# ut-amrl/nautilus

Measured on AMD Instinct MI355X. Metric: loop-closure candidate pairs/sec (1081-beam), higher is better.
Workload: dtype u16

## Files before the change

nautilus_amd/csrc/nhip_bnb.hip:

```cpp
#include <atomic>
#include <mutex>
#include <type_traits>
#include <vector>

#ifndef NHIP_BNB_INSTR
#define NHIP_BNB_INSTR 0
#endif
#if NHIP_BNB_INSTR
#define csm_bnb_kernel csm_bnb_kernel_instr
#define csm_bnb_rot_kernel csm_bnb_rot_kernel_instr
#define launchers_product launchers_instr
#define BNB_STATS(P) ((P).stats)
#define BNB_TIMELINE(P) ((P).timeline)
#else
#define BNB_STATS(P) (static_cast<unsigned long long *>(nullptr))
#define BNB_TIMELINE(P) (static_cast<unsigned long long *>(nullptr))
#endif

#include "nhip_bnb_params.h"
#include "nhip_bnb_wave.h"
#include "nhip_bnb_origin.h"
#include "nhip_bnb_bounds.h"
#include "nhip_bnb_exact.h"

// ... 239 lines not shown
      for (int q = 0; q < 12; q++) sb[q] = 0xffffffffu;
    }
    uint32_t mk0 = 0u, mk1 = 0u;
#pragma unroll 1
    for (int t = 0; t < len; t++) {
      const int b = b0 + t;
      if (b < 64) m0 &= ~(1ull << b);
      else m1 &= ~(1ull << (b - 64));
      const uint32_t ub = (uint32_t)__builtin_amdgcn_readlane((int)(b < 64 ? u0 : u1), b & 63);
      if (ub < best_sum_cached<GLOBAL>(best, bcopy)) continue;
      const uint32_t s0 = t == 0 ? sb[0] : (t == 1 ? sb[4] : sb[8]), s1 = t == 0 ? sb[1] : (t == 1 ? sb[5] : sb[9]);
      const uint32_t s2 = t == 0 ? sb[2] : (t == 1 ? sb[6] : sb[10]), s3 = t == 0 ? sb[3] : (t == 1 ? sb[7] : sb[11]);
      if (BNB_STATS(P)) t_mark = clock64();
      process_candidate_c<CB, GLOBAL, PAIR>(P, rsrc, pitch8, rsrc16, org, nch, C.n_pts, k, Y, X0 + t, s0, s1, s2, s3, lane, best,
                                      bcopy, n_work, t, mk0, mk1);
      if (BNB_STATS(P)) clk.eval += clock64() - t_mark;
      if (done && wave_leader(lane)) done[b] = 0u;
    }
    if (PAIR && (mk0 | mk1) != 0u) {
      if (BNB_STATS(P)) t_mark = clock64();
      strip_sub_blocks<CB, GLOBAL>(P, rsrc, pitch8, rsrc16, org, nch, C.n_pts, k, Y, X0, sb, mk0, mk1, lane, best, bcopy, n_work);
      if (BNB_STATS(P)) clk.eval += clock64() - t_mark;
    }
  }
}

__device__ __forceinline__ void read_entry(const RotEntry *ent, int32_t *pair, int32_t *k, unsigned long long *m0,
                                           unsigned long long *m1) {
  const unsigned long long w0 = ent->w[0], w1 = ent->w[1], w2 = ent->w[2], w3 = ent->w[3];
  *pair = (int32_t)(w0 >> 24);
  *k = (int32_t)(w0 & 0xffffffull);
  *m0 = w1 | (w2 << 41);
  *m1 = (w2 >> 23) | (w3 << 18);
}

__device__ __forceinline__ void pair_context(const BnbParams &P, int32_t pair, PairCtx *C) {
  const int32_t src = P.pair_src[pair], slot = P.pair_slot[pair];
  const int32_t beg = P.offsets[src];
  C->grid = P.grids + (size_t)slot * P.slot_bytes;
  C->pts = P.xy + beg;
  C->n_pts = P.offsets[src + 1] - beg;
  C->cx = P.pair_origin ? P.pair_origin[2 * pair] : 0;
  C->cy = P.pair_origin ? P.pair_origin[2 * pair + 1] : 0;
  C->pair = pair;
}

template <int CB, bool POOL_LDS, bool BY_ROT, bool SPLIT = false>
__global__ __launch_bounds__(SPLIT ? 64 * SPLIT_WAVES : BNB_THREADS, SPLIT ? SPLIT_WAVES / 2 : 4) void csm_bnb_kernel(BnbParams P) {
  constexpr int WAVES = SPLIT ? SPLIT_WAVES : BNB_WAVES, THREADS = 64 * WAVES;
  constexpr int QSPACE = lds_qspace(SPLIT);
  extern __shared__ __align__(16) uint8_t smem[];
  uint8_t *s_pool = smem;
  uint32_t *s_org = reinterpret_cast<uint32_t *>(smem);
  uint32_t *s_U = reinterpret_cast<uint32_t *>(smem + P.lds_first);
  unsigned long long *s_queue = reinterpret_cast<unsigned long long *>(s_U + (size_t)P.n_theta * 128);
  LdsTail *s_tail = reinterpret_cast<LdsTail *>(s_queue + QSPACE);
  unsigned long long *s_best = &s_tail->best, *s_slow = &s_tail->slow;
  uint32_t *s_cnt = s_tail->cnt, *s_qn = s_cnt + LDS_QN, *s_qhead = s_cnt + LDS_QHEAD, *s_top = &s_tail->top;
  uint32_t *s_list = reinterpret_cast<uint32_t *>(s_queue);
  static_assert(BNB_WAVES * LIST_ENTRIES * 4 <= QCAP * 4, "the run lists fit the first half of the queue");
  unsigned long long *s_kmax = s_queue + (SPLIT ? WAVES * LIST_ENTRIES / 2 : QCAP / 2);
  uint32_t *s_order = reinterpret_cast<uint32_t *>(s_kmax + MAX_ROT);
  static_assert(SPLIT_WAVES * LIST_ENTRIES * 4 + MAX_ROT * 12 <= QSPACE_SPLIT * 8 && MAX_ROT * 12 <= QCAP * 4, "lists, maxima and order fit");

  const uint32_t bid = blockIdx.x;
  const int32_t pair = (int32_t)((bid & 7u) * (uint32_t)P.pairs_per_xcd + (bid >> 3));
  if ((int32_t)(bid >> 3) >= P.pairs_per_xcd || pair >= P.n_pairs) return;
  const int lane = threadIdx.x & 63, wave = threadIdx.x >> 6;

  int32_t src = P.pair_src[pair], slot = P.pair_slot[pair];
  const bool ids_ok = pair_ids_ok(P.ids, src, slot, pair + P.pair_base, threadIdx.x == 0);
  if (!ids_ok) src = slot = 0;
  const int32_t beg = ids_ok ? P.offsets[src] : 0, n_pts = ids_ok ? P.offsets[src + 1] - beg : 0;
  const float2 *pts = P.xy + beg;
  const uint8_t *grid = P.grids + (size_t)slot * P.slot_bytes;
  const int32_t cx = P.pair_origin ? P.pair_origin[2 * pair] : 0;
  const int32_t cy = P.pair_origin ? P.pair_origin[2 * pair + 1] : 0;
  const bool centre_ok = (abs(cx) + P.hx <= P.max_shift) && (abs(cy) + P.hy <= P.max_shift);
  if (BY_ROT != (n_pts <= 64 * OCL && (uint32_t)P.rows < ORG_LIMIT && !P.general_all)) return;

  const int32_t gfloor = gate_floor(P.gate, n_pts);
  const unsigned long long fkey = gate_floor_key(gfloor);
  unsigned long long *const stats_g = NHIP_BNB_INSTR ? P.stats : nullptr;
  const long long t_start = BNB_STATS(P) ? clock64() : 0;
  if (BNB_TIMELINE(P) && threadIdx.x == 0 && pair < BNB_STATS_PAIRS) BNB_TIMELINE(P)[4 * pair] = wall_clock64();
  if (threadIdx.x == 0) {
    *s_slow = 0ull;
    *s_best = fkey;
    s_cnt[0] = s_cnt[3] = s_cnt[4] = s_cnt[5] = 0u;
    s_top[0] = 0u;
    *s_qn = 0u;
    *s_qhead = 0u;
  }
  if (!centre_ok || n_pts <= 0) {
    if (threadIdx.x == 0) P.keys[pair] = fkey;
    return;
  }
  const RotationTerms terms = rotation_terms_of_wave<WAVES>(P, pair, wave, lane);
  if (POOL_LDS) {
    const uint4 *gp = reinterpret_cast<const uint4 *>(grid + P.grid_bytes + P.skip_bytes);
    uint4 *sp = reinterpret_cast<uint4 *>(s_pool);
    const int32_t n16 = (int32_t)(P.pool_bytes / 16);
    for (int32_t i = threadIdx.x; i < n16; i += 4 * THREADS) {
      uint4 v[4];
#pragma unroll
      for (int j = 0; j < 4; j++) v[j] = gp[min(i + j * THREADS, n16 - 1)];
#pragma unroll
      for (int j = 0; j < 4; j++)
        if (i + j * THREADS < n16) sp[i + j * THREADS] = v[j];
    }
  }
  const __amdgpu_buffer_rsrc_t prs = uniform_rsrc(grid + P.grid_bytes + P.skip_bytes, P.pool_bytes);
  float cfs, sfs;
  rotation_of(terms, &cfs, &sfs);
  __syncthreads();

  const uint32_t scale = CB == 1 ? 1u : 257u;
  unsigned long long wbest = 0ull;
  PointSlots slots;
  prime_slots(pts, wave < P.n_theta ? n_pts : 0, lane, slots);
  int32_t mine = 0;
  for (int32_t k = wave; k < P.n_theta; k += WAVES, mine++) {
    const float cf = __int_as_float(__builtin_amdgcn_readlane(__float_as_int(cfs), mine));
    const float sf = __int_as_float(__builtin_amdgcn_readlane(__float_as_int(sfs), mine));
    uint32_t umax = 0u;
    uint32_t tot[2];
    coarse_rotation<POOL_LDS>(P, s_pool, prs, pts, n_pts, slots, cf, sf, cx, cy, lane, s_list + wave * LIST_ENTRIES, tot);
    if (lane < 128 - NB * NB) s_U[k * 128 + NB * NB + lane] = 0u;
#pragma unroll
    for (int i = 0; i < 2; i++) {
      int Y, X;
      if (!slot_block(lane + 64 * i, &Y, &X)) continue;
      const uint32_t u = (Y < P.nby && X < P.nbx) ? tot[i] * scale : 0u;
      const int b = NB * Y + X;
      s_U[k * 128 + b] = u;
      umax = u > umax ? u : umax;
      const unsigned long long cand = ((unsigned long long)u << 32) | (uint32_t)((k << 8) | b);
      wbest = cand > wbest ? cand : wbest;
    }
    if (BY_ROT) {
      umax = wave_max(umax);
      if (wave_leader(lane)) s_kmax[k] = ((unsigned long long)umax << 32) | (uint32_t)k;
    }
  }
  wbest = wave_max_u64(wbest);
  if (gfloor > 0) {
    if (wave_leader(lane)) atomicMax(s_top, (uint32_t)(wbest >> 32));
    __syncthreads();
    if (*s_top < (uint32_t)gfloor) {
      if (threadIdx.x == 0) {
        P.keys[pair] = fkey;
        if (stats_g) {
          atomicAdd(&stats_g[1], (unsigned long long)(P.n_theta * P.nbx * P.nby));
          atomicAdd(&stats_g[15], 1ull);
        }
      }
      return;
    }
    if ((uint32_t)(wbest >> 32) < (uint32_t)gfloor) wbest = 0ull;
  }
  uint32_t n_work[N_WORK] = {};
  PairCtx C;
  C.grid = grid;
  C.pts = pts;
  C.n_pts = n_pts;
  C.cx = cx;
  C.cy = cy;
  C.pair = pair;
  if (BY_ROT) {
    __syncthreads();
    uint32_t *org = s_org + wave * ORG_WAVE + lane;
    PhaseClocks clk = {0, 0, 0, 0u, 0u, 0u};
    long long t_busy = 0, t_wall = 0;
    const long long t_phase1 = BNB_STATS(P) ? clock64() : 0;
    if (BNB_TIMELINE(P) && threadIdx.x == 0 && pair < BNB_STATS_PAIRS) BNB_TIMELINE(P)[4 * pair + 1] = wall_clock64();
    const uint32_t xcd = bid & 7u;
    bool handed_over = false;
    enum { SEED, OWN };
    int state = SEED;
    bool heavy = false;
    for (;;) {
      bool have = false;
      int32_t k = 0;
      uint32_t u0 = 0u, u1 = 0u;
      unsigned long long m0 = 0ull, m1 = 0ull;
      uint32_t *done = nullptr;
      if (state == SEED) {
        if ((uint32_t)(wbest >> 32) != 0u) {
          const int32_t v = (int32_t)(wbest & 0xffu);
          const uint32_t ub = (uint32_t)(wbest >> 32);
          k = (int32_t)((uint32_t)wbest >> 8);
          u0 = v == lane ? ub : 0u;
          u1 = v == lane + 64 ? ub : 0u;
          m0 = v < 64 ? 1ull << v : 0ull;
          m1 = v < 64 ? 0ull : 1ull << (v - 64);
          done = s_U + k * 128;
          have = true;
        }
      } else if (state == OWN) {
        const int32_t rank = (int32_t)wave_fetch_add(s_qhead, 1u, lane);
        if (rank >= P.n_theta) break;
        k = (int32_t)s_order[rank];
        u0 = s_U[k * 128 + lane];
        u1 = s_U[k * 128 + 64 + lane];
        const uint32_t bsum = best_sum<false>(s_best);
        m0 = __ballot(u0 != 0u && u0 >= bsum);
        m1 = __ballot(u1 != 0u && u1 >= bsum && lane + 64 < NB * NB);
        if ((m0 | m1) == 0ull) continue;
        if (heavy && (uint32_t)rank >= P.keep_ranks) {
          const uint32_t lx = (xcd + (uint32_t)rank) & 7u;
          const uint32_t e = wave_fetch_add(P.rot_count + 8 * lx, 1u, lane);
          if (e < P.rot_cap) {
            if (lane < 4) {
              const unsigned long long M41 = (1ull << 41) - 1ull;
              const unsigned long long word = lane == 0   ? ((unsigned long long)(uint32_t)pair << 24) | (uint32_t)k
                                              : lane == 1 ? (m0 & M41)
                                              : lane == 2 ? ((m0 >> 41) | (m1 << 23)) & M41
                                                          : (m1 >> 18);
              P.rot_list[(size_t)lx * P.rot_cap + e].w[lane] = word;
            }
            handed_over = true;
            continue;
          }
        }
        have = true;
      }
      if (have) rotation_pass<CB, false, false>(P, C, k, u0, u1, m0, m1, lane, s_best, done, org, n_work, clk);
      if (state == SEED) {
        __syncthreads();
        if (BNB_TIMELINE(P) && threadIdx.x == 0 && pair < BNB_STATS_PAIRS) BNB_TIMELINE(P)[4 * pair + 2] = wall_clock64();
        if (BNB_STATS(P)) {
          t_busy = clock64();
          t_wall = wall_clock64();
        }
        for (int32_t kk = threadIdx.x; kk < P.n_theta; kk += THREADS) {
          const unsigned long long mine = s_kmax[kk];
          int32_t rank = 0;
          for (int32_t j = 0; j < P.n_theta; j++) rank += s_kmax[j] > mine ? 1 : 0;
          s_order[rank] = (uint32_t)kk;
        }
        if (P.rot_list || SPLIT) {
          const uint32_t bsum = best_sum<false>(s_best);
          uint32_t mine = 0u;
          for (int32_t kk = wave; kk < P.n_theta; kk += WAVES) {
            const uint32_t c0 = s_U[kk * 128 + lane], c1 = s_U[kk * 128 + 64 + lane];
            mine += (uint32_t)__builtin_popcountll(__ballot(c0 != 0u && c0 >= bsum)) +
                    (uint32_t)__builtin_popcountll(__ballot(c1 != 0u && c1 >= bsum && lane + 64 < NB * NB));
          }
          if (wave_leader(lane)) atomicAdd(s_qn, mine);
        }
        __syncthreads();
        if (SPLIT) {
          const uint32_t bsum = best_sum<false>(s_best);
          uint32_t *rows = P.ps_rows + (size_t)pair * (size_t)P.n_theta * 128u;
          uint32_t live = 0u;
          for (int32_t r = wave; r < P.n_theta; r += WAVES) {
            const uint32_t kk = s_order[r];
            const uint32_t kmax = (uint32_t)(s_kmax[kk] >> 32);
            if (kmax == 0u || kmax < bsum) break;
            live = (uint32_t)r + 1u;
            const uint32_t w1 = lane == 62 ? kmax : (lane == 63 ? kk : s_U[kk * 128 + 64 + lane]);
            rows[(size_t)r * 128u + lane] = s_U[kk * 128 + lane];
            rows[(size_t)r * 128u + 64 + lane] = w1;
          }
          if (live && wave_leader(lane)) atomicMax(s_qhead, live);
          __syncthreads();
          if (threadIdx.x == 0) {
            P.ps_count[pair] = *s_qn;
            P.ps_live[pair] = *s_qhead;
            P.ps_next[pair] = 0u;
          }
          break;
        }
        heavy = P.rot_list && *s_qn >= P.heavy_min;
        state = OWN;
      }
    }
    if (BNB_STATS(P) && lane == 0) {
      const long long now = clock64();
      atomicAdd(&BNB_STATS(P)[4], (unsigned long long)(now - t_busy));
      atomicAdd(&BNB_STATS(P)[11], (unsigned long long)(wall_clock64() - t_wall));
      flush_stats(BNB_STATS(P), nullptr, pair, &clk);
      atomicMax(s_slow, (unsigned long long)(now - t_busy));
      if (wave == 0) {
        atomicAdd(&BNB_STATS(P)[9], (unsigned long long)(t_busy - t_phase1));
        atomicAdd(&BNB_STATS(P)[10], (unsigned long long)(t_phase1 - t_start));
        if (handed_over) atomicAdd(&BNB_STATS(P)[12], 1ull);
      }
    }
  } else {
  if ((uint32_t)(wbest >> 32) != 0u) {
      const int32_t k = (int32_t)((uint32_t)wbest >> 8), v = (int32_t)(wbest & 0xffu);
      const int Y = v / NB, X = v - NB * Y;
      float cf, sf;
      rotation_k(P, pair, k, &cf, &sf);
      const unsigned long long key = eval_block<CB>(P, grid, pts, n_pts, cf, sf, cx, cy, k, Y, X, lane);
      if (wave_leader(lane)) {
        atomicMax(s_best, key);
        s_U[k * 128 + v] = 0u;
      }
      n_work[0]++;
    }
    __syncthreads();
    for (int32_t k = wave; k < P.n_theta; k += BNB_WAVES) {
  #pragma unroll
      for (int i = 0; i < 2; i++) {
        const uint32_t u = s_U[k * 128 + lane + 64 * i];
        const uint32_t bsum = (uint32_t)(*(volatile unsigned long long *)s_best >> 32);
        bool cand = u != 0u && u >= bsum;
        const unsigned long long m = __ballot(cand);
        if (m == 0ull) continue;
        const uint32_t base = wave_fetch_add(s_qn, (uint32_t)__builtin_popcountll(m), lane);
        const uint32_t pos = base + (uint32_t)__builtin_popcountll(m & ((1ull << lane) - 1ull));
        const unsigned long long entry = ((unsigned long long)u << 32) | (uint32_t)((k << 8) | (lane + 64 * i));
        if (cand && pos < (uint32_t)QCAP) s_queue[pos] = entry;
        unsigned long long over = __ballot(cand && pos >= (uint32_t)QCAP);
        while (over) {
          const int j = (int)__builtin_ctzll(over);
          over &= over - 1ull;
          const uint32_t lo = (uint32_t)__builtin_amdgcn_readlane((int)(uint32_t)entry, j);
          const uint32_t hi = (uint32_t)__builtin_amdgcn_readlane((int)(uint32_t)(entry >> 32), j);
          if (hi >= best_sum<false>(s_best))
            process_candidate<CB>(P, C, (int32_t)(lo >> 8), (int32_t)(lo & 0xffu), lane, s_best, n_work);
        }
      }
    }
    __syncthreads();
    {
      const uint32_t qn = min(*s_qn, (uint32_t)QCAP);
      for (;;) {
        const uint32_t i = wave_fetch_add(s_qhead, 1u, lane);
        if (i >= qn) break;
        const unsigned long long entry = s_queue[i];
        if ((uint32_t)(entry >> 32) >= best_sum<false>(s_best))
          process_candidate<CB>(P, C, (int32_t)((uint32_t)entry >> 8), (int32_t)(entry & 0xffu), lane, s_best, n_work);
      }
    }
}
  if (stats_g && lane == 0) {
    atomicAdd(&s_cnt[0], n_work[0]);
    atomicAdd(&s_cnt[3], n_work[1]);
    atomicAdd(&s_cnt[4], n_work[2]);
    atomicAdd(&s_cnt[5], n_work[3]);
    flush_stats(stats_g, nullptr, pair, nullptr, n_work + 4);
  }
  __syncthreads();
  if (threadIdx.x == 0) {
    P.keys[pair] = *s_best;
    if (BNB_TIMELINE(P) && pair < BNB_STATS_PAIRS) {
      uint32_t hw;
      asm volatile("s_getreg_b32 %0, hwreg(HW_REG_HW_ID)" : "=s"(hw));
      uint32_t xcc;
      asm volatile("s_getreg_b32 %0, hwreg(HW_REG_XCC_ID)" : "=s"(xcc));
      BNB_TIMELINE(P)[4 * pair + 3] = (wall_clock64() & 0xfffffffffffull) | ((unsigned long long)((hw >> 8) & 0xffu) << 44) |
                                      ((unsigned long long)(xcc & 0xfu) << 52);
    }
    if (BNB_STATS(P) && BY_ROT) atomicAdd(&BNB_STATS(P)[8], *s_slow);
    if (stats_g) {
      const uint32_t n_all[4] = {s_cnt[0], s_cnt[3], s_cnt[4], s_cnt[5]};
      flush_stats(stats_g, n_all, pair, nullptr);
      atomicAdd(&stats_g[1], (unsigned long long)(P.n_theta * P.nbx * P.nby));
    }
  }
}
// ... 262 lines not shown
```

nautilus_amd/csrc/nhip_bnb_bounds.h:

```cpp
#pragma once
#include <type_traits>

#include "nhip_bnb_origin.h"

namespace nhip {
namespace {

constexpr uint32_t LANE_WEIGHT = 64u;

struct PointSlots {
  float2 q0, q1;
};
__device__ __forceinline__ void prime_slots(const float2 *pts, int32_t n_pts, int lane, PointSlots &S) {
  S.q0 = S.q1 = make_float2(0.f, 0.f);
  if (n_pts > 0) {
    const int32_t last = n_pts - 1;
    S.q0 = pts[min(lane, last)];
    __builtin_amdgcn_sched_barrier(0);
    S.q1 = pts[min(64 + lane, last)];
  }
}

template <bool POOL_LDS>
__device__ __forceinline__ void coarse_rotation(const BnbParams &P, const uint8_t *pool, __amdgpu_buffer_rsrc_t prs,
                                                const float2 *pts, int32_t n_pts, PointSlots &S, float cf, float sf,
                                                int32_t cx, int32_t cy, int lane, uint32_t *list, uint32_t (&tot)[2]) {
  const int32_t DP = P.pool_pitch;
  const uint32_t zero_a = (uint32_t)(((P.rows + BNB_B - 1) / BNB_B) * DP);
  tot[0] = tot[1] = 0u;
  uint32_t E[NB][3], O[NB][3];
#pragma unroll
  for (int y = 0; y < NB; y++)
#pragma unroll
    for (int d = 0; d < 3; d++) E[y][d] = O[y][d] = 0u;
  uint32_t head = 0u, tail = 0u;
  uint32_t reduced = 0u;
  uint32_t weight = 0u;

  auto gather = [&](uint32_t a, uint32_t cnt) {
    const uint32_t se = __umul24(a & 3u, 0x10001u) + 0x0c020c00u, so = se + 0x00010001u;
    const uint32_t *q = reinterpret_cast<const uint32_t *>(pool + (a & ~3u));
    auto add_row = [&](int y, uint32_t w0, uint32_t w1, uint32_t w2, uint32_t w3) {
      E[y][0] += __umul24(__builtin_amdgcn_perm(w1, w0, se), cnt); O[y][0] += __umul24(__builtin_amdgcn_perm(w1, w0, so), cnt);
      E[y][1] += __umul24(__builtin_amdgcn_perm(w2, w1, se), cnt); O[y][1] += __umul24(__builtin_amdgcn_perm(w2, w1, so), cnt);
      E[y][2] += __umul24(__builtin_amdgcn_perm(w3, w2, se), cnt); O[y][2] = mad24(__builtin_amdgcn_perm(w3, w2, so), cnt, O[y][2]);
    };
    auto load_row = [&](int y, uint32_t &w0, uint32_t &w1, uint32_t &w2, uint32_t &w3) {
      if (POOL_LDS) {
        const uint32_t *row = q + (y * DP) / 4;
        w0 = row[0]; w1 = row[1]; w2 = row[2]; w3 = row[3];
      } else {
        const u32x4 r4 = __builtin_amdgcn_raw_buffer_load_b128(prs, (int)((a & ~3u) + (uint32_t)(y * DP)), 0, 0);
        w0 = r4.x; w1 = r4.y; w2 = r4.z; w3 = r4.w;
      }
    };
    uint32_t n0, n1, n2, n3;
    load_row(0, n0, n1, n2, n3);
#pragma unroll
    for (int y = 0; y < NB; y++) {
      const uint32_t w0 = n0, w1 = n1, w2 = n2, w3 = n3;
      if (y + 1 < NB) load_row(y + 1, n0, n1, n2, n3);
      __builtin_amdgcn_sched_barrier(0);
      add_row(y, w0, w1, w2, w3);
      __builtin_amdgcn_sched_barrier(0);
    }
  };
  auto reduce = [&]() {
    uint32_t R[64];
#pragma unroll
    for (int y = 0; y < 10; y++)
#pragma unroll
      for (int d = 0; d < 3; d++) {
        R[6 * y + d] = E[y][d];
        R[6 * y + 3 + d] = O[y][d];
      }
    R[5] = (O[0][2] & 0xffffu) | (O[10][1] << 16);
    R[11] = (O[1][2] & 0xffffu) | (O[10][1] & 0xffff0000u);
    R[17] = (O[2][2] & 0xffffu) | (O[10][2] << 16);
    R[60] = E[10][0];
    R[61] = E[10][1];
    R[62] = E[10][2];
    R[63] = O[10][0];
    rs_step<64, 1>(R, lane & 1);
    rs_step<32, 2>(R, lane & 2);
    uint32_t V[32];
#pragma unroll
    for (int i = 0; i < 16; i++) {
      V[2 * i] = R[i] & 0xffffu;
      V[2 * i + 1] = R[i] >> 16;
    }
    rs_step<32, 4>(V, lane & 4);
    rs_step<16, 8>(V, lane & 8);
    rs_step<8, 16>(V, lane & 16);
    rs_step<4, 32>(V, lane & 32);
    tot[0] += V[0];
    tot[1] += V[1];
#pragma unroll
    for (int y = 0; y < NB; y++)
#pragma unroll
      for (int d = 0; d < 3; d++) E[y][d] = O[y][d] = 0u;
  };

  auto feed = [&](uint32_t a, int32_t c, bool more) {
    if (more) {
      const bool live = c + lane < n_pts;
      const uint32_t prev = (uint32_t)__builtin_amdgcn_update_dpp((int)a, (int)a, 0x138 , 0xF, 0xF, false);
      const bool is_head = (lane & 63) == 0 || a != prev;
      const unsigned long long H = __builtin_amdgcn_uicmp(a, prev, 33 ) | 1ull;
      uint32_t cnt = (uint32_t)(c + lane) & 127u;
      cnt += 1u;
      const int32_t n_live = n_pts - c;
      const unsigned long long He = H & (n_live >= 64 ? ~0ull : (1ull << n_live) - 1ull);
      if (is_head && live) {
        const uint32_t before = __builtin_amdgcn_mbcnt_hi((uint32_t)(He >> 32), __builtin_amdgcn_mbcnt_lo((uint32_t)He, 0u));
        list[(tail + before) & (LIST_ENTRIES - 1)] = a | ((cnt - 1u) << RUN_SHIFT);
      }
      tail += (uint32_t)__builtin_popcountll(He);
      __builtin_amdgcn_fence(__ATOMIC_RELEASE, "wavefront");
      __builtin_amdgcn_wave_barrier();
    }
    if (!more) {
      if (lane == 0) list[tail & (LIST_ENTRIES - 1)] = ((uint32_t)n_pts & 127u) << RUN_SHIFT;
      __builtin_amdgcn_fence(__ATOMIC_RELEASE, "wavefront");
      __builtin_amdgcn_wave_barrier();
    }
    for (;;) {
      const uint32_t avail = tail - head;
      if (avail < 65u && more) break;
      const bool last = avail == 0u;
      const bool mine = (uint32_t)lane < avail;
      const uint32_t entry = mine ? list[(head + (uint32_t)lane) & (LIST_ENTRIES - 1)] : zero_a;
      const uint32_t ea = entry & ((1u << RUN_SHIFT) - 1u);
      const uint32_t next = mine ? list[(head + (uint32_t)lane + 1u) & (LIST_ENTRIES - 1)] : 0u;
      const uint32_t cnt = mine ? ((next >> RUN_SHIFT) - (entry >> RUN_SHIFT)) & 127u : 0u;
      uint32_t left = avail;
      asm("" : "+s"(left));
      if (head != reduced && (left == 0u || __builtin_amdgcn_uicmp(weight + cnt, LANE_WEIGHT, 34 ) != 0ull)) {
        reduce();
        reduced = head;
        weight = 0u;
      }
      if (last) break;
      gather(ea, cnt);
      weight += cnt;
      head += avail < 64u ? avail : 64u;
      __builtin_amdgcn_wave_barrier();
    }
  };

  auto offsets = [&](float2 pt, int32_t c) {
    uint32_t a = zero_a;
    if (c + lane < n_pts) {
      int32_t prow, pcol;
      window_origin<true>(pt, cf, sf, P, cx, cy, &prow, &pcol);
      a = __umul24((uint32_t)prow >> 3, (uint32_t)DP) + ((uint32_t)pcol >> 3);
    }
    return a;
  };
  constexpr int PD = 2;
  if (n_pts > 0) {
    const int32_t last = n_pts - 1;
    for (int32_t c = 0; c < n_pts; c += 64 * PD) {
      const int32_t cn = c + 64 * PD < n_pts ? c + 64 * PD : 0;
      {
        float2 pt = S.q0;
        asm volatile("" : "+v"(pt.x), "+v"(pt.y));
        S.q0 = pts[min(cn + lane, last)];
        feed(offsets(pt, c), c, true);
      }
      {
        float2 pt = S.q1;
        asm volatile("" : "+v"(pt.x), "+v"(pt.y));
        S.q1 = pts[min(cn + 64 + lane, last)];
        if (c + 64 < n_pts) feed(offsets(pt, c + 64), c + 64, true);
      }
    }
  }
  feed(zero_a, 0, false);
}

__device__ __forceinline__ bool slot_block(int v, int *Y, int *X) {
  const int lane = v & 63, i = v >> 6;
  const int r = 32 * i + 16 * ((lane >> 5) & 1) + 8 * ((lane >> 4) & 1) + 4 * ((lane >> 3) & 1) + 2 * ((lane >> 1) & 1) + (lane & 1);
  const int f = (lane >> 2) & 1;
  if (r >= 60) {
    *Y = 10;
    *X = r == 63 ? 1 + 2 * f : 4 * (r - 60) + 2 * f;
    return true;
  }
  const int y = r / 6, d = r % 6;
  if (d == 5 && f == 1) {
    *Y = 10;
    *X = 5 + 2 * y;
    return y < 3;
  }
  *Y = y;
  *X = d < 3 ? 4 * d + 2 * f : 4 * (d - 3) + 1 + 2 * f;
  return true;
}

__device__ __forceinline__ void sub_bounds(const BnbParams &P, __amdgpu_buffer_rsrc_t p4, const float2 *pts, int32_t n_pts,
                                           float cf, float sf, int32_t cx, int32_t cy, int32_t Y, int32_t X, int lane,
                                           uint32_t scale, uint32_t (&out)[4]) {
  const int32_t DP = P.pool4_pitch;
  uint32_t A[4] = {0u, 0u, 0u, 0u};
  constexpr int U = 4;
  for (int32_t c = 0; c < n_pts; c += 64 * U) {
    uint32_t a[U];
    u32x2 w[U];
#pragma unroll
    for (int u = 0; u < U; u++) {
      const int32_t idx = c + 64 * u + lane;
      a[u] = 0u;
      if (idx < n_pts) {
        int32_t prow, pcol;
        window_origin(pts[idx], cf, sf, P, cx, cy, &prow, &pcol);
        a[u] = (uint32_t)(((prow >> 2) + 2 * Y) * DP + 2 * ((pcol >> 2) + 2 * X));
      }
      w[u] = __builtin_amdgcn_raw_buffer_load_b64(p4, (int)(a[u] & ~3u), 0, 0);
    }
#pragma unroll
    for (int u = 0; u < U; u++) {
      const uint32_t n = idx_guard(c + 64 * u + lane < n_pts, __builtin_amdgcn_alignbit(w[u].y, w[u].x, (a[u] & 2u) * 8u));
      A[0] += n & 0xffu;
      A[2] += (n >> 8) & 0xffu;
      A[1] += (n >> 16) & 0xffu;
      A[3] += n >> 24;
    }
  }
#pragma unroll
  for (int m = 1; m < 64; m <<= 1) {
#pragma unroll
    for (int q = 0; q < 4; q++) A[q] += shfl_xor_u32(A[q], m);
  }
#pragma unroll
  for (int q = 0; q < 4; q++) out[q] = A[q] * scale;
}

// ... 95 lines not shown
```

nautilus_amd/csrc/nhip_bnb_origin.h:

```cpp
#pragma once
#include "nhip_bnb_params.h"
#include "nhip_bnb_wave.h"

namespace nhip {
namespace {

using namespace bnb;

template <bool LEAN = false>
__device__ __forceinline__ void window_origin(float2 q, float cf, float sf, const BnbParams &P, int32_t cx, int32_t cy,
                                              int32_t *prow, int32_t *pcol) {
  const float xr = __fsub_rn(__fmul_rn(cf, q.x), __fmul_rn(sf, q.y));
  const float yr = __fadd_rn(__fmul_rn(sf, q.x), __fmul_rn(cf, q.y));
  const int32_t half = P.S / 2;
  const bool finite __attribute__((unused)) = (fabsf(xr) < 1e9f) && (fabsf(yr) < 1e9f);
  int32_t ix, iy;
  const float mx = __fmul_rn(xr, P.inv_res_f), my = __fmul_rn(yr, P.inv_res_f);
  const float fx = floorf(mx), fy = floorf(my);
  if (LEAN) {
    const float rx = __fsub_rn(mx, fx), ry = __fsub_rn(my, fy);
    const float dx = fminf(rx, __fsub_rn(1.0f, rx)), dy = fminf(ry, __fsub_rn(1.0f, ry));
    const float tx = __fmul_rn(fabsf(mx), 0x1p-22f), ty = __fmul_rn(fabsf(my), 0x1p-22f);
    const unsigned long long slow = __builtin_amdgcn_fcmpf(dx, tx, 13 ) | __builtin_amdgcn_fcmpf(dy, ty, 13 );
    ix = (int32_t)fx;
    iy = (int32_t)fy;
    const int32_t kx = half + cx - P.hx + P.pad, ky = half + cy - P.hy + P.pad;
    if (slow != 0ull) {
      const bool near_x = !(dx > tx), near_y = !(dy > ty);
      const bool big = (int)!(fabsf(mx) < 0x1p22f) | (int)!(fabsf(my) < 0x1p22f);
      const int32_t nx = (int32_t)rintf(mx), ny = (int32_t)rintf(my);
      const bool stay = (int)big | ((int)near_x & (int)(((nx + kx) & 7) == 0)) | ((int)near_y & (int)(((ny + ky) & 7) == 0));
      if (__builtin_amdgcn_ballot_w64(stay) != 0ull) {
        if (stay) {
          const double xd = (double)xr, yd = (double)yr;
          const bool fin = (fabs(xd) < 1e9) && (fabs(yd) < 1e9);
          ix = (int32_t)fmin(fmax(floor_quotient(xd, P.res, P.inv_res), -2147483000.0), 2147483000.0);
          iy = (int32_t)fmin(fmax(floor_quotient(yd, P.res, P.inv_res), -2147483000.0), 2147483000.0);
          if (!fin) ix = iy = -2147483000;
        }
      }
    }
    const int32_t lo_x = -P.hx - 1 - half - cx, lo_y = -P.hy - 1 - half - cy;
    ix = min(max(ix, lo_x), P.S + P.hx - half - cx);
    iy = min(max(iy, lo_y), P.S + P.hy - half - cy);
    *pcol = ix + kx;
    *prow = iy + ky;
    return;
  }
  const float rx = __fsub_rn(mx, fx), ry = __fsub_rn(my, fy);
  const bool near = fminf(rx, __fsub_rn(1.0f, rx)) <= __fmul_rn(fabsf(mx), 0x1p-22f) ||
                    fminf(ry, __fsub_rn(1.0f, ry)) <= __fmul_rn(fabsf(my), 0x1p-22f);
  ix = (int32_t)fx;
  iy = (int32_t)fy;
  if (__builtin_amdgcn_ballot_w64(near && finite) != 0ull) {
    if (near && finite) {
      ix = (int32_t)fmin(fmax(floor_quotient((double)xr, P.res, P.inv_res), -2147483000.0), 2147483000.0);
      iy = (int32_t)fmin(fmax(floor_quotient((double)yr, P.res, P.inv_res), -2147483000.0), 2147483000.0);
    }
  }
  ix = min(max(ix, -P.hx - 1 - half - cx), P.S + P.hx - half - cx);
  iy = min(max(iy, -P.hy - 1 - half - cy), P.S + P.hy - half - cy);
  const int32_t col = finite ? half + ix + cx : -P.hx - 1, row = finite ? half + iy + cy : -P.hy - 1;
  *pcol = col - P.hx + P.pad;
  *prow = row - P.hy + P.pad;
}

typedef uint32_t u32x2 __attribute__((ext_vector_type(2)));
typedef uint32_t u32x3 __attribute__((ext_vector_type(3)));
typedef uint32_t u32x4 __attribute__((ext_vector_type(4)));

__device__ __forceinline__ __amdgpu_buffer_rsrc_t uniform_rsrc(const void *base, int64_t bytes) {
  const uint64_t a = reinterpret_cast<uint64_t>(base);
  const uint32_t lo = (uint32_t)__builtin_amdgcn_readfirstlane((int)(uint32_t)a);
  const uint32_t hi = (uint32_t)__builtin_amdgcn_readfirstlane((int)(uint32_t)(a >> 32));
  const int n = __builtin_amdgcn_readfirstlane((int)(bytes < 0x7fffffffll ? bytes : 0x7fffffffll));
  return __builtin_amdgcn_make_buffer_rsrc(reinterpret_cast<void *>(((uint64_t)hi << 32) | lo), 0, n, 0x00020000);
}

__device__ __forceinline__ uint32_t idx_guard(bool live, uint32_t v) { return live ? v : 0u; }

struct RotationTerms {
  double c0, s0, cd, sd;
};
__device__ __forceinline__ RotationTerms rotation_terms(const BnbParams &P, int32_t pair, int32_t k) {
  RotationTerms T;
  T.c0 = P.rot0_cs[2 * pair];
  T.s0 = P.rot0_cs[2 * pair + 1];
  const int32_t kd = k + (P.pair_kbase ? P.pair_kbase[pair] : 0);
  T.cd = P.delta_cs[2 * kd];
  T.sd = P.delta_cs[2 * kd + 1];
  return T;
}
__device__ __forceinline__ void rotation_of(const RotationTerms &T, float *cf, float *sf) {
  *cf = __double2float_rn(__dsub_rn(__dmul_rn(T.c0, T.cd), __dmul_rn(T.s0, T.sd)));
  *sf = __double2float_rn(__dadd_rn(__dmul_rn(T.s0, T.cd), __dmul_rn(T.c0, T.sd)));
}
__device__ __forceinline__ void rotation_k(const BnbParams &P, int32_t pair, int32_t k, float *cf, float *sf) {
  rotation_of(rotation_terms(P, pair, k), cf, sf);
}

template <int WAVES>
__device__ __forceinline__ RotationTerms rotation_terms_of_wave(const BnbParams &P, int32_t pair, int32_t wave, int lane) {
  static_assert(MAX_ROT <= 64 * WAVES, "a wave's rotations fit its lanes");
  RotationTerms T = {1.0, 0.0, 1.0, 0.0};
  if (wave < P.n_theta) {
    const int32_t mine = (P.n_theta - 1 - wave) / WAVES + 1;
    T = rotation_terms(P, pair, wave + WAVES * min(lane, mine - 1));
  }
  return T;
}

__device__ __forceinline__ void patch_origin(const BnbParams &P, bool live, float2 q, float cf, float sf, int32_t cx,
                                             int32_t cy, int32_t Y, int32_t X, uint32_t *g, uint32_t *sh) {
  *g = 0u;
  *sh = 0u;
  if (live) {
    int32_t prow, pcol;
    window_origin(q, cf, sf, P, cx, cy, &prow, &pcol);
    const int32_t col = pcol + BNB_B * X;
    *g = (uint32_t)((prow + BNB_B * Y) * P.pitch + (col & ~3));
    *sh = (uint32_t)(col & 3) * 8u;
  }
}


constexpr int ORG_COL_SHIFT = 6, ORG_ROW_SHIFT = 19;
__device__ __forceinline__ uint32_t org_row(uint32_t o) { return o >> ORG_ROW_SHIFT; }
__device__ __forceinline__ uint32_t org_col(uint32_t o) { return (o >> ORG_COL_SHIFT) & (ORG_LIMIT - 1u); }
__device__ __forceinline__ uint32_t org_cnt(uint32_t o) { return (o & 63u) + 1u; }

__device__ __forceinline__ uint32_t origin_of(const uint32_t *org, int c) { return c < OCL ? org[64 * c] : 0u; }

constexpr uint32_t RUN_KEY_MASK = (~0u << (ORG_ROW_SHIFT + 2)) | (((ORG_LIMIT >> 2) - 1u) << (ORG_COL_SHIFT + 2));
__device__ __forceinline__ uint32_t run_row2(uint32_t e) { return e >> (ORG_ROW_SHIFT + 2); }
__device__ __forceinline__ uint32_t run_col2(uint32_t e) { return (e >> (ORG_COL_SHIFT + 2)) & ((ORG_LIMIT >> 2) - 1u); }
__device__ __forceinline__ uint32_t run_cnt(uint32_t e) { return e & 127u; }
enum : int32_t { RUNS_NONE = 0, RUNS_FIELD = -1, RUNS_FULL = -2 };

template <bool RUNS = false, bool RING = RUNS>
__device__ __forceinline__ int32_t cache_origins(const BnbParams &P, const float2 *pts, int32_t n_pts, float cf, float sf,
                                                 int32_t cx, int32_t cy, int lane, uint32_t *org, bool merged,
                                                 uint32_t *runs = nullptr, bool want_runs = false,
                                                 int32_t *run_chunks = nullptr) {
  uint32_t *base = org - lane;
  const bool with_runs = RUNS && want_runs;
  if (RUNS) *run_chunks = RUNS_NONE;
  for (int merge = merged ? 1 : 0; merge >= 0; merge--) {
// ... 116 lines not shown
```

Before: 1.820 million.

## Compute coarse pooled cell directly with prescaled rotation and frame constants

Replaces the per-point window-origin computation in the coarse bound pass with a pooled chain. The rotation and grid frame are pre-scaled by 1/8 and the offset is folded in, so two FMAs plus a floor and a med3 clamp yield the 8x-pooled cell index directly instead of going through full-resolution rounding and shifts. It keeps a tolerance-based fallback to the exact double-precision path near cell boundaries, with scalarised constants via readfirstlane. Instrumentation timers are narrowed to 32-bit. The risk is subtle correctness at pooled boundaries if the tolerance bounds are wrong.

```diff
diff --git a/nautilus_amd/csrc/nhip_bnb.hip b/nautilus_amd/csrc/nhip_bnb.hip
--- a/nautilus_amd/csrc/nhip_bnb.hip
+++ b/nautilus_amd/csrc/nhip_bnb.hip
@@ -345,7 +345,7 @@
   const int32_t gfloor = gate_floor(P.gate, n_pts);
   const unsigned long long fkey = gate_floor_key(gfloor);
   unsigned long long *const stats_g = NHIP_BNB_INSTR ? P.stats : nullptr;
-  const long long t_start = BNB_STATS(P) ? clock64() : 0;
+  const uint32_t t_start = BNB_STATS(P) ? (uint32_t)clock64() : 0u;
   if (BNB_TIMELINE(P) && threadIdx.x == 0 && pair < BNB_STATS_PAIRS) BNB_TIMELINE(P)[4 * pair] = wall_clock64();
   if (threadIdx.x == 0) {
     *s_slow = 0ull;
@@ -376,6 +376,7 @@
   const __amdgpu_buffer_rsrc_t prs = uniform_rsrc(grid + P.grid_bytes + P.skip_bytes, P.pool_bytes);
   float cfs, sfs;
   rotation_of(terms, &cfs, &sfs);
+  const pooled::Frame frame = uniform_frame(pooled::frame(P.S, P.pad, P.hx, P.hy, cx, cy));
   __syncthreads();
 
   const uint32_t scale = CB == 1 ? 1u : 257u;
@@ -386,9 +387,10 @@
   for (int32_t k = wave; k < P.n_theta; k += WAVES, mine++) {
     const float cf = __int_as_float(__builtin_amdgcn_readlane(__float_as_int(cfs), mine));
     const float sf = __int_as_float(__builtin_amdgcn_readlane(__float_as_int(sfs), mine));
+    const pooled::Rotation rot = uniform_rotation(pooled::rotation(cf, sf, P.inv_res));
     uint32_t umax = 0u;
     uint32_t tot[2];
-    coarse_rotation<POOL_LDS>(P, s_pool, prs, pts, n_pts, slots, cf, sf, cx, cy, lane, s_list + wave * LIST_ENTRIES, tot);
+    coarse_rotation<POOL_LDS>(P, s_pool, prs, pts, n_pts, slots, cf, sf, rot, frame, cx, cy, lane, s_list + wave * LIST_ENTRIES, tot);
     if (lane < 128 - NB * NB) s_U[k * 128 + NB * NB + lane] = 0u;
 #pragma unroll
     for (int i = 0; i < 2; i++) {
@@ -434,8 +436,8 @@
     __syncthreads();
     uint32_t *org = s_org + wave * ORG_WAVE + lane;
     PhaseClocks clk = {0, 0, 0, 0u, 0u, 0u};
-    long long t_busy = 0, t_wall = 0;
-    const long long t_phase1 = BNB_STATS(P) ? clock64() : 0;
+    uint32_t t_busy = 0u, t_wall = 0u;
+    const uint32_t t_phase1 = BNB_STATS(P) ? (uint32_t)clock64() : 0u;
     if (BNB_TIMELINE(P) && threadIdx.x == 0 && pair < BNB_STATS_PAIRS) BNB_TIMELINE(P)[4 * pair + 1] = wall_clock64();
     const uint32_t xcd = bid & 7u;
     bool handed_over = false;
@@ -493,8 +495,8 @@
         __syncthreads();
         if (BNB_TIMELINE(P) && threadIdx.x == 0 && pair < BNB_STATS_PAIRS) BNB_TIMELINE(P)[4 * pair + 2] = wall_clock64();
         if (BNB_STATS(P)) {
-          t_busy = clock64();
-          t_wall = wall_clock64();
+          t_busy = (uint32_t)clock64();
+          t_wall = (uint32_t)wall_clock64();
         }
         for (int32_t kk = threadIdx.x; kk < P.n_theta; kk += THREADS) {
           const unsigned long long mine = s_kmax[kk];
@@ -540,9 +542,9 @@
       }
     }
     if (BNB_STATS(P) && lane == 0) {
-      const long long now = clock64();
+      const uint32_t now = (uint32_t)clock64();
       atomicAdd(&BNB_STATS(P)[4], (unsigned long long)(now - t_busy));
-      atomicAdd(&BNB_STATS(P)[11], (unsigned long long)(wall_clock64() - t_wall));
+      atomicAdd(&BNB_STATS(P)[11], (unsigned long long)((uint32_t)wall_clock64() - t_wall));
       flush_stats(BNB_STATS(P), nullptr, pair, &clk);
       atomicMax(s_slow, (unsigned long long)(now - t_busy));
       if (wave == 0) {
diff --git a/nautilus_amd/csrc/nhip_bnb_bounds.h b/nautilus_amd/csrc/nhip_bnb_bounds.h
--- a/nautilus_amd/csrc/nhip_bnb_bounds.h
+++ b/nautilus_amd/csrc/nhip_bnb_bounds.h
@@ -24,7 +24,8 @@
 template <bool POOL_LDS>
 __device__ __forceinline__ void coarse_rotation(const BnbParams &P, const uint8_t *pool, __amdgpu_buffer_rsrc_t prs,
                                                 const float2 *pts, int32_t n_pts, PointSlots &S, float cf, float sf,
-                                                int32_t cx, int32_t cy, int lane, uint32_t *list, uint32_t (&tot)[2]) {
+                                                const pooled::Rotation &R, const pooled::Frame &F, int32_t cx, int32_t cy,
+                                                int lane, uint32_t *list, uint32_t (&tot)[2]) {
   const int32_t DP = P.pool_pitch;
   const uint32_t zero_a = (uint32_t)(((P.rows + BNB_B - 1) / BNB_B) * DP);
   tot[0] = tot[1] = 0u;
@@ -148,12 +149,13 @@
     }
   };
 
+  const uint32_t org_a = (uint32_t)(F.lo8y * DP + F.lo8x);
   auto offsets = [&](float2 pt, int32_t c) {
     uint32_t a = zero_a;
     if (c + lane < n_pts) {
-      int32_t prow, pcol;
-      window_origin<true>(pt, cf, sf, P, cx, cy, &prow, &pcol);
-      a = __umul24((uint32_t)prow >> 3, (uint32_t)DP) + ((uint32_t)pcol >> 3);
+      int32_t prow8, pcol8;
+      pooled_origin(pt, cf, sf, R, F, P, cx, cy, &prow8, &pcol8);
+      a = __umul24((uint32_t)prow8, (uint32_t)DP) + ((uint32_t)pcol8 + org_a);
     }
     return a;
   };
diff --git a/nautilus_amd/csrc/nhip_bnb_origin.h b/nautilus_amd/csrc/nhip_bnb_origin.h
--- a/nautilus_amd/csrc/nhip_bnb_origin.h
+++ b/nautilus_amd/csrc/nhip_bnb_origin.h
@@ -1,5 +1,6 @@
 #pragma once
 #include "nhip_bnb_params.h"
+#include "nhip_bnb_pooled.h"
 #include "nhip_bnb_wave.h"
 
 namespace nhip {
@@ -7,46 +8,15 @@
 
 using namespace bnb;
 
-template <bool LEAN = false>
 __device__ __forceinline__ void window_origin(float2 q, float cf, float sf, const BnbParams &P, int32_t cx, int32_t cy,
                                               int32_t *prow, int32_t *pcol) {
   const float xr = __fsub_rn(__fmul_rn(cf, q.x), __fmul_rn(sf, q.y));
   const float yr = __fadd_rn(__fmul_rn(sf, q.x), __fmul_rn(cf, q.y));
   const int32_t half = P.S / 2;
-  const bool finite __attribute__((unused)) = (fabsf(xr) < 1e9f) && (fabsf(yr) < 1e9f);
+  const bool finite = (fabsf(xr) < 1e9f) && (fabsf(yr) < 1e9f);
   int32_t ix, iy;
   const float mx = __fmul_rn(xr, P.inv_res_f), my = __fmul_rn(yr, P.inv_res_f);
   const float fx = floorf(mx), fy = floorf(my);
-  if (LEAN) {
-    const float rx = __fsub_rn(mx, fx), ry = __fsub_rn(my, fy);
-    const float dx = fminf(rx, __fsub_rn(1.0f, rx)), dy = fminf(ry, __fsub_rn(1.0f, ry));
-    const float tx = __fmul_rn(fabsf(mx), 0x1p-22f), ty = __fmul_rn(fabsf(my), 0x1p-22f);
-    const unsigned long long slow = __builtin_amdgcn_fcmpf(dx, tx, 13 ) | __builtin_amdgcn_fcmpf(dy, ty, 13 );
-    ix = (int32_t)fx;
-    iy = (int32_t)fy;
-    const int32_t kx = half + cx - P.hx + P.pad, ky = half + cy - P.hy + P.pad;
-    if (slow != 0ull) {
-      const bool near_x = !(dx > tx), near_y = !(dy > ty);
-      const bool big = (int)!(fabsf(mx) < 0x1p22f) | (int)!(fabsf(my) < 0x1p22f);
-      const int32_t nx = (int32_t)rintf(mx), ny = (int32_t)rintf(my);
-      const bool stay = (int)big | ((int)near_x & (int)(((nx + kx) & 7) == 0)) | ((int)near_y & (int)(((ny + ky) & 7) == 0));
-      if (__builtin_amdgcn_ballot_w64(stay) != 0ull) {
-        if (stay) {
-          const double xd = (double)xr, yd = (double)yr;
-          const bool fin = (fabs(xd) < 1e9) && (fabs(yd) < 1e9);
-          ix = (int32_t)fmin(fmax(floor_quotient(xd, P.res, P.inv_res), -2147483000.0), 2147483000.0);
-          iy = (int32_t)fmin(fmax(floor_quotient(yd, P.res, P.inv_res), -2147483000.0), 2147483000.0);
-          if (!fin) ix = iy = -2147483000;
-        }
-      }
-    }
-    const int32_t lo_x = -P.hx - 1 - half - cx, lo_y = -P.hy - 1 - half - cy;
-    ix = min(max(ix, lo_x), P.S + P.hx - half - cx);
-    iy = min(max(iy, lo_y), P.S + P.hy - half - cy);
-    *pcol = ix + kx;
-    *prow = iy + ky;
-    return;
-  }
   const float rx = __fsub_rn(mx, fx), ry = __fsub_rn(my, fy);
   const bool near = fminf(rx, __fsub_rn(1.0f, rx)) <= __fmul_rn(fabsf(mx), 0x1p-22f) ||
                     fminf(ry, __fsub_rn(1.0f, ry)) <= __fmul_rn(fabsf(my), 0x1p-22f);
@@ -63,6 +33,46 @@
   const int32_t col = finite ? half + ix + cx : -P.hx - 1, row = finite ? half + iy + cy : -P.hy - 1;
   *pcol = col - P.hx + P.pad;
   *prow = row - P.hy + P.pad;
+}
+
+__device__ __forceinline__ float scalar_copy(float v) {
+  int i;
+  asm volatile("s_nop 1\n\tv_readfirstlane_b32 %0, %1\n\ts_nop 1" : "=s"(i) : "v"(__float_as_int(v)));
+  return __int_as_float(i);
+}
+__device__ __forceinline__ pooled::Frame uniform_frame(const pooled::Frame &F) {
+  return pooled::Frame{scalar_copy(F.k8x), scalar_copy(F.k8y), scalar_copy(F.tol_k), scalar_copy(F.hi8x), scalar_copy(F.hi8y), F.lo8x, F.lo8y};
+}
+__device__ __forceinline__ pooled::Rotation uniform_rotation(const pooled::Rotation &R) {
+  return pooled::Rotation{scalar_copy(R.c8), scalar_copy(R.s8), scalar_copy(R.tol_m)};
+}
+__device__ __forceinline__ void pooled_origin(float2 q, float cf, float sf, const pooled::Rotation &R, const pooled::Frame &F,
+                                              const BnbParams &P, int32_t cx, int32_t cy, int32_t *prow8, int32_t *pcol8) {
+  const pooled::Chain C = pooled::chain(q.x, q.y, R, F);
+  const unsigned long long slow = __builtin_amdgcn_fcmpf(fabsf(C.dx), C.tol, 13 ) | __builtin_amdgcn_fcmpf(fabsf(C.dy), C.tol, 13 );
+  int32_t ex = pooled::entry(C.fx, F.hi8x), ey = pooled::entry(C.fy, F.hi8y);
+  if (slow != 0ull) {
+    if ((int)!(fabsf(C.dx) > C.tol) | (int)!(fabsf(C.dy) > C.tol)) {
+      const float xr = __fsub_rn(__fmul_rn(cf, q.x), __fmul_rn(sf, q.y));
+      const float yr = __fadd_rn(__fmul_rn(sf, q.x), __fmul_rn(cf, q.y));
+      const double xd = (double)xr, yd = (double)yr;
+      const bool fin = (fabs(xd) < 1e9) && (fabs(yd) < 1e9);
+      int32_t ix = (int32_t)fmin(fmax(floor_quotient(xd, P.res, P.inv_res), -2147483000.0), 2147483000.0);
+      int32_t iy = (int32_t)fmin(fmax(floor_quotient(yd, P.res, P.inv_res), -2147483000.0), 2147483000.0);
+      if (!fin) ix = iy = -2147483000;
+      int32_t S = P.S, hx = P.hx, hy = P.hy, pad = P.pad, ox = cx, oy = cy;
+#if NHIP_BNB_INSTR
+      asm volatile("" : "+s"(S), "+s"(hx), "+s"(hy), "+s"(pad), "+s"(ox), "+s"(oy));
+#endif
+      const int32_t half = S / 2;
+      ix = min(max(ix, -hx - 1 - half - ox), S + hx - half - ox);
+      iy = min(max(iy, -hy - 1 - half - oy), S + hy - half - oy);
+      ex = ((ix + half + ox - hx + pad) >> 3) - ((pad - 2 * hx - 1) >> 3);
+      ey = ((iy + half + oy - hy + pad) >> 3) - ((pad - 2 * hy - 1) >> 3);
+    }
+  }
+  *pcol8 = ex;
+  *prow8 = ey;
 }
 
 typedef uint32_t u32x2 __attribute__((ext_vector_type(2)));
diff --git a/nautilus_amd/csrc/nhip_bnb_pooled.h b/nautilus_amd/csrc/nhip_bnb_pooled.h
--- /dev/null
+++ b/nautilus_amd/csrc/nhip_bnb_pooled.h
@@ -0,0 +1,67 @@
+#pragma once
+#include <math.h>
+#include <stdint.h>
+
+#if defined(__HIPCC__)
+#define NHIP_POOLED_FN __host__ __device__ __forceinline__
+#else
+#define NHIP_POOLED_FN inline
+#endif
+
+namespace nhip {
+namespace pooled {
+
+struct Rotation {
+  float c8, s8, tol_m;
+};
+NHIP_POOLED_FN Rotation rotation(float cf, float sf, double inv_res) {
+  Rotation R;
+  R.c8 = (float)((double)cf * inv_res * 0.125);
+  R.s8 = (float)((double)sf * inv_res * 0.125);
+  R.tol_m = 0x1.8p-22f * fmaxf(fabsf(R.c8), fabsf(R.s8));
+  return R;
+}
+
+struct Frame {
+  float k8x, k8y, tol_k, hi8x, hi8y;
+  int32_t lo8x, lo8y;
+};
+NHIP_POOLED_FN Frame frame(int32_t S, int32_t pad, int32_t hx, int32_t hy, int32_t cx, int32_t cy) {
+  Frame F;
+  const int32_t kx = S / 2 + cx - hx + pad, ky = S / 2 + cy - hy + pad;
+  F.lo8x = (pad - 2 * hx - 1) >> 3;
+  F.lo8y = (pad - 2 * hy - 1) >> 3;
+  F.k8x = (float)(kx - 8 * F.lo8x) * 0.125f;
+  F.k8y = (float)(ky - 8 * F.lo8y) * 0.125f;
+  F.tol_k = 0x1.8p-23f * fmaxf(fabsf(F.k8x), fabsf(F.k8y)) + 0x1p-40f;
+  F.hi8x = (float)(((S + pad) >> 3) - F.lo8x);
+  F.hi8y = (float)(((S + pad) >> 3) - F.lo8y);
+  return F;
+}
+
+struct Chain {
+  float fx, fy, dx, dy, tol;
+};
+NHIP_POOLED_FN Chain chain(float x, float y, const Rotation &R, const Frame &F) {
+  Chain C;
+  const float tx = fmaf(R.c8, x, fmaf(-R.s8, y, F.k8x));
+  const float ty = fmaf(R.s8, x, fmaf(R.c8, y, F.k8y));
+  C.fx = floorf(tx);
+  C.fy = floorf(ty);
+  C.dx = tx - rintf(tx);
+  C.dy = ty - rintf(ty);
+  C.tol = fmaf(fabsf(x) + fabsf(y), R.tol_m, F.tol_k);
+  return C;
+}
+NHIP_POOLED_FN bool near(const Chain &C) { return !(fabsf(C.dx) > C.tol) || !(fabsf(C.dy) > C.tol); }
+
+NHIP_POOLED_FN int32_t entry(float f, float hi8) {
+#if defined(__HIP_DEVICE_COMPILE__)
+  return (int32_t)__builtin_amdgcn_fmed3f(f, 0.0f, hi8);
+#else
+  return (int32_t)fminf(fmaxf(f, 0.0f), hi8);
+#endif
+}
+
+}
+}
```

Result: no change. 1.837 million, median of 6 (+0.9%).
